# fx-erick/uncertainty-vit

Hardware: AMD Instinct MI355X
Metric: pretrain images/sec (ViT-B/16 224, bs=128/GPU) (higher is better)
Workload: dtype bf16

## Files before the change

include/uvit.h:

```cpp
#ifndef UVIT_H
#define UVIT_H
#include <stddef.h>
#include <stdint.h>

#ifdef __cplusplus
extern "C" {
#endif

#define UVIT_VERSION 100
#define UVIT_MAX_DEPTH 64

typedef struct uvit_engine uvit_engine;
typedef void* uvit_stream;

typedef struct uvit_config {
    int32_t img_size, patch_size, in_chans, embed_dim, depth, num_heads, mlp_hidden;
    int32_t use_shared_rel_pos_bias;
    int32_t use_abs_pos_emb;
    int32_t batch;
    float ln_eps;
    float attn_drop_rate;
    float drop_path_rate;
    int32_t bias_chunk;
    int32_t two_stream;
// ... 91 lines not shown

typedef struct uvit_gemm_epilogue {
    void* out; void* out2; const float* bias; const float* bias2; const float* gamma; const float* resid;
    const float* rowscale; const void* aux; const int64_t* mask; const float* mask_token;
    int32_t ldo, tokens, patches;
    int32_t row0;
} uvit_gemm_epilogue;
enum { UVIT_EPI_BF16 = 0, UVIT_EPI_QKV = 1, UVIT_EPI_GELU = 2, UVIT_EPI_RESID = 3, UVIT_EPI_F32 = 4,
       UVIT_EPI_PATCH = 5, UVIT_EPI_DGELU = 6, UVIT_EPI_QKV_ELU = 7,
       UVIT_EPI_GELU_DG = 8,
       UVIT_EPI_MULAUX = 9 };

int uvit_op_gemm_nt(int mode, const void* A_bf16, const void* W_bf16, int M, int N, int K, int lda, int ldw,
                    const uvit_gemm_epilogue* epi, uvit_stream stream);
int uvit_op_gemm_nt_tuned(int mode, const void* A_bf16, const void* W_bf16, int M, int N, int K, int lda, int ldw,
                          const uvit_gemm_epilogue* epi, const uvit_tuning* tune, int* tail_rows, uvit_stream stream);
typedef struct uvit_gemm_nt_plan_info { int32_t kernel, rows, grid, tail_rows; } uvit_gemm_nt_plan_info;
int uvit_op_gemm_nt_plan(int mode, int M, int N, int K, int lda, int ldw, int ldo, int row_list,
                         const uvit_tuning* tuning, int num_cu, uvit_gemm_nt_plan_info* out);
int uvit_op_gemm_nt_sched(int mode, const void* A_bf16, const void* W_bf16, int M, int N, int K, int lda, int ldw,
                          const uvit_gemm_epilogue* epi, const uvit_tuning* tune, uint32_t* tile_counters, uvit_stream stream);
int uvit_op_gemm_tn(const void* Y_bf16, const void* X_bf16, int M, int N, int K, int ldy, int ldx, float* C, int ldc,
                    const uvit_tuning* tune, uvit_stream stream);
typedef struct uvit_wgrad_problem {
    const void* Y_bf16; const void* X_bf16; float* C; float* bias; float* bias2;
    int32_t bias_end, bias2_begin, M, N, K, ldy, ldx, ldc;
} uvit_wgrad_problem;
int uvit_op_wgrad_group(const uvit_wgrad_problem* problems, int count, const uvit_tuning* tune, uvit_stream stream);
int uvit_op_attn_fwd(const void* qkv, const float* biasP, void* out, float* lse, int B, int H, int N, int NP,
                     float scale, float p_drop, uint32_t seed, uint32_t layer, uvit_stream stream);
int64_t uvit_op_attn_bwd_ws_bytes(int B, int H, int N);
int uvit_op_attn_bwd(const void* qkv, const void* o_fwd, const void* d_o, const float* biasP, const float* lse,
                           float* delta, void* dqkv, float* dbias_slab, int accumulate_slab, void* ds_workspace, int B, int H,
                           int N, int NP, float scale, float p_drop, uint32_t seed, uint32_t layer, uvit_stream stream);
int uvit_op_attn_fwd_hd(const void* qkv, const float* biasP, void* out, float* lse, int B, int H, int N, int NP, int head_dim,
                        float scale, float p_drop, uint32_t seed, uint32_t layer, uvit_stream stream);
int uvit_op_attn_bwd_hd(const void* qkv, const void* o_fwd, const void* d_o, const float* biasP, const float* lse,
                        float* delta, void* dqkv, float* dbias_slab, int accumulate_slab, void* ds_workspace, int B, int H,
                        int N, int NP, int head_dim, float scale, float p_drop, uint32_t seed, uint32_t layer, uvit_stream stream);
int uvit_op_attn2_fwd(const void* qkv_m, const void* qkv_c, const float* biasP, void* out_m, void* out_c, float* lse, int B, int H,
                      int N, int NP, float scale, float p_drop, uint32_t seed, uint32_t layer, uvit_stream stream);
int64_t uvit_op_attn2_bwd_ws_bytes(int B, int H, int N);
int uvit_op_attn2_bwd(const void* qkv_m, const void* qkv_c, const void* o_m, const void* o_c, const void* d_m, const void* d_c,
                      const float* biasP, const float* lse, float* delta, void* dqkv_m, void* dqkv_c, float* dbias_slab,
                      int accumulate_slab, void* ds_workspace, int B, int H, int N, int NP, float scale, float p_drop, uint32_t seed,
                      uint32_t layer, uvit_stream stream);
int uvit_op_relpos_gather(const float* table, const int32_t* index, float* biasP, int H, int N, int NP, uvit_stream stream);
int uvit_op_relpos_scatter(const float* slab, int nslab, const int32_t* index, float* dtable, int H, int N, int NP,
                           uvit_stream stream);
int uvit_op_ln_fwd(const float* x, const float* w, const float* b, void* y_bf16, float* mean, float* rstd, int M, int C,
                   float eps, uvit_stream stream);
int uvit_op_ln_bwd(const void* dy_bf16, const float* x, const float* mean, const float* rstd, const float* w,
                   const float* dres, float* dx, float* dw, float* db, int M, int C, uvit_stream stream);
int uvit_op_ema(float* ema, const float* params, void* ema_bf16, int64_t n, float decay, uvit_stream stream);
int uvit_op_sumsq(const float* g, int64_t n, double* out, uvit_stream stream);
int uvit_op_adamw(float* p, const float* g, float* m, float* v, void* p_bf16, int64_t n, int64_t n_decay, float lr,
                  float wd, float b1, float b2, float eps, int step, const double* sumsq, float max_norm,
                  float grad_scale, float* gnorm_out, uvit_stream stream);
int uvit_op_smooth_l1(const float* out, const float* target, const int32_t* count_dev, float beta, int l2,
                      float loss_scale, float* loss, void* dout_bf16, int Mmax, int C, uvit_stream stream);
int uvit_op_wasserstein_loss(const float* out_m, const float* out_c, const float* tgt_m, const float* tgt_c,
                             const int32_t* count_dev, float lam, float loss_scale, float* scratch, float* loss,
                             void* dout_m_bf16, void* dout_c_bf16, int Mmax, int C, uvit_stream stream);
int uvit_op_target_accum(const float* x, const int32_t* rowidx, const int32_t* count, float* acc, int first, int Mmax,
                         int C, float eps, uvit_stream stream);
int uvit_op_variance_loss(const float* out, const int32_t* count_dev, float w, float margin, float loss_scale, float* scratch,
                          float* loss, float* std_loss0_out, void* dout_bf16, int Mmax, int C, uvit_stream stream);
int uvit_op_target_finalize(float* acc, const int32_t* count, int n_layers, int post_ln, int Mmax, int C, float eps,
                            uvit_stream stream);
int uvit_op_mask_compact(const int64_t* mask, int32_t* rowidx, int32_t* count, int B, int P, uvit_stream stream);
int uvit_op_synth_batch(float* images, int64_t* mask, int B, int chans, int img_size, int patches, int n_mask, uint32_t seed,
                        uint32_t it, uvit_stream stream);
int uvit_op_im2col(const float* img, void* cols_bf16, int B, int Cin, int img_size, int patch, uvit_stream stream);
int uvit_op_droppath(float* scales, const float* rates_dev, int depth, int B, uint32_t seed, uint32_t step,
                     uvit_stream stream);
int uvit_op_cast_bf16(const float* src, void* dst_bf16, int64_t n, uvit_stream stream);

#define UVIT_AUG_LANCZOS 1
#define UVIT_AUG_BILINEAR 2
#define UVIT_AUG_BICUBIC 3
#define UVIT_AUG_HAMMING 5
#define UVIT_AUG_BRIGHTNESS 0
#define UVIT_AUG_CONTRAST 1
#define UVIT_AUG_SATURATION 2
typedef struct uvit_augment_desc {
    int64_t offset;
    int32_t h, w;
    int32_t flip;
    int32_t crop_x, crop_y, crop_w, crop_h;
    int32_t resize_w, resize_h;
    int32_t win_x, win_y;
    int32_t filter;
    int32_t n_jitter;
    int32_t jitter_op[3];
    float jitter_factor[3];
    int32_t reserved;
} uvit_augment_desc;
int64_t uvit_op_augment_ws_bytes(const uvit_augment_desc* desc, int B, int S);
int uvit_op_augment_batch(const uint8_t* pixels, int64_t pixel_bytes, const uvit_augment_desc* desc, int B, int S, const float* mean,
                          const float* std, float* out, void* workspace, int64_t ws_bytes, uvit_stream stream);

int64_t uvit_op_probe_pool_ws_bytes(int B, int N, int C);
int uvit_op_probe_pool_norm(const float* x, float* feat, float* scratch, int B, int N, int C, float eps, uvit_stream stream);
int uvit_op_probe_logits(const float* feat, const float* W, const float* bias, float* logits, int B, int K, int C, uvit_stream stream);
int uvit_op_probe_ce(const float* logits, const int64_t* labels, float smoothing, float* dlogits, float* row_loss, float* loss_out,
                     int32_t* top1_top5, int B, int K, uvit_stream stream);
// ... 15 lines not shown
```

uncertainty-vit_amd/csrc/engine.hip:

```cpp
#include <hip/hip_runtime.h>
#include <math.h>
#include <stdio.h>
#include <stdlib.h>
#include <string.h>

#include <string>
#include <vector>

#include "../../include/uvit.h"
#include "common.h"
#include "uvit_internal.h"

#define CHECK(x) do { int _rc = (x); if (_rc) return _rc; } while (0)
#define NREP 32
#define RP(off) (e->grep + ((off) - e->lo.n_decay))
#define HIPCHECK(x) do { if ((x) != hipSuccess) return UVIT_ERR_LAUNCH; } while (0)
#define GEMM_NT(...) uvit_gemm_nt_launch(__VA_ARGS__, &e->tune)
#define GEMM_TN(...) uvit_gemm_tn_launch(__VA_ARGS__, &e->tune)
#define GEMM_TN_GROUP(...) uvit_gemm_tn_group_launch(__VA_ARGS__, &e->tune)

struct LayerOff { size_t n1w, n1b, qkvw, qb[2], vb[2], projw[2], projb[2], g1, n2w, n2b, fc1w, fc1b, fc2w, fc2b, g2, cqkvw; };
struct Layout {
    size_t cls[2], mask_tok[2], pew[2], peb[2], relt, normw, normb, lmw[2], lmb[2], pos;
    LayerOff L[UVIT_MAX_DEPTH];
    size_t n_total, n_decay, n_live;
    std::vector<uvit_layout_entry> entries;
};

static size_t align64(size_t x) { return (x + 63) & ~(size_t)63; }

static int cfg_ok(const uvit_config* c) {
    if (!c) return UVIT_ERR_ARG;
    if (c->depth < 1 || c->depth > UVIT_MAX_DEPTH || c->num_heads < 1) return UVIT_ERR_SHAPE;
    if (c->embed_dim != c->num_heads * 64 && (c->two_stream || c->embed_dim != c->num_heads * 80)) return UVIT_ERR_SHAPE;
    if (c->embed_dim % 64 || c->mlp_hidden % 64 || c->patch_size % 8 || c->img_size % c->patch_size) return UVIT_ERR_SHAPE;
    if ((c->in_chans * c->patch_size * c->patch_size) % 64) return UVIT_ERR_SHAPE;
    const int g = c->img_size / c->patch_size;
    if (g * g + 1 > 208 || c->batch < 1) return UVIT_ERR_SHAPE;
    if (c->use_abs_pos_emb && c->two_stream) return UVIT_ERR_SHAPE;
    return UVIT_OK;
}

static void build_layout(const uvit_config* c, Layout& lo) {
    const int64_t C = c->embed_dim, Hd = c->mlp_hidden, g = c->img_size / c->patch_size;
    size_t off = 0;
    auto add = [&](const std::string& name, std::vector<int64_t> shape, int decay) -> size_t {
        uvit_layout_entry e;
        memset(&e, 0, sizeof(e));
        snprintf(e.name, sizeof(e.name), "%s", name.c_str());
        e.offset = (int64_t)off; e.ndim = (int)shape.size(); e.decay = decay; e.numel = 1;
        for (size_t i = 0; i < shape.size(); ++i) { e.shape[i] = shape[i]; e.numel *= shape[i]; }
        lo.entries.push_back(e);
        const size_t at = off;
        off = align64(off + (size_t)e.numel);
        return at;
    };
    auto blk = [](int i, const char* s) { return "blocks." + std::to_string(i) + "." + s; };
    const bool two = c->two_stream != 0;
    lo.mask_tok[0] = add("mask_token", {1, 1, C}, 1);
    if (two) lo.mask_tok[1] = add("cov_mask_token", {1, 1, C}, 1);
    if (two) lo.cls[1] = add("cov_cls_token", {1, 1, C}, 1);
    if (c->use_shared_rel_pos_bias) lo.relt = add("rel_pos_bias.relative_position_bias_table", {(2 * g - 1) * (2 * g - 1) + 3, c->num_heads}, 1);
    else lo.relt = (size_t)-1;
    lo.pew[0] = add("patch_embed.proj.weight", {C, c->in_chans, c->patch_size, c->patch_size}, 1);
// ... 1050 lines not shown
    return UVIT_OK;
}
extern "C" int uvit_op_attn_fwd_hd(const void* qkv, const float* biasP, void* out, float* lse, int B, int H, int N, int NP, int head_dim,
                                   float scale, float p_drop, uint32_t seed, uint32_t layer, uvit_stream st) {
    if (!qkv || !out || !lse) return UVIT_ERR_ARG;
    if (head_dim != 64 && head_dim != 80) return UVIT_ERR_SHAPE;
    return uvit_attn_fwd_launch(qkv, biasP, out, lse, B, H, N, NP, scale, p_drop, seed, layer, S(st), nullptr, head_dim);
}
extern "C" int uvit_op_attn_bwd_hd(const void* qkv, const void* o_fwd, const void* d_o, const float* biasP, const float* lse,
                                   float* delta, void* dqkv, float* slab, int acc, void* ds_ws, int B, int H, int N, int NP, int head_dim,
                                   float scale, float p_drop, uint32_t seed, uint32_t layer, uvit_stream st) {
    if (!qkv || !o_fwd || !d_o || !lse || !delta || !dqkv || (slab && !ds_ws)) return UVIT_ERR_ARG;
    if (head_dim != 64 && head_dim != 80) return UVIT_ERR_SHAPE;
    CHECK(uvit_attn_bwd_fused_launch(qkv, o_fwd, d_o, biasP, lse, delta, dqkv, ds_ws, slab != nullptr, B, H, N, NP, scale, p_drop, seed, layer,
                                     S(st), nullptr, head_dim));
    if (slab) CHECK(uvit_attn_dbias_reduce_launch(ds_ws, slab, acc, B, H, N, NP, S(st)));
    return UVIT_OK;
}
extern "C" int uvit_op_attn2_fwd(const void* qkv_m, const void* qkv_c, const float* biasP, void* out_m, void* out_c, float* lse, int B,
                                 int H, int N, int NP, float scale, float p_drop, uint32_t seed, uint32_t layer, uvit_stream st) {
    if (!qkv_m || !qkv_c || !out_m || !out_c || !lse) return UVIT_ERR_ARG;
    return uvit_attn2_fwd_launch(qkv_m, qkv_c, biasP, out_m, out_c, lse, B, H, N, NP, scale, p_drop, seed, layer, S(st));
}
extern "C" int64_t uvit_op_attn2_bwd_ws_bytes(int B, int H, int N) {
    if (B <= 0 || H <= 0 || N <= 0) return UVIT_ERR_SHAPE;
    return (int64_t)uvit_attn2_bwd_ws_bytes(B, H, N);
}
extern "C" int uvit_op_attn2_bwd(const void* qkv_m, const void* qkv_c, const void* o_m, const void* o_c, const void* d_m, const void* d_c,
                                 const float* biasP, const float* lse, float* delta, void* dqkv_m, void* dqkv_c, float* slab, int acc,
                                 void* ds_ws, int B, int H, int N, int NP, float scale, float p_drop, uint32_t seed, uint32_t layer,
                                 uvit_stream st) {
    if (!qkv_m || !qkv_c || !o_m || !o_c || !d_m || !d_c || !lse || !delta || !dqkv_m || !dqkv_c || (slab && !ds_ws)) return UVIT_ERR_ARG;
    CHECK(uvit_attn2_bwd_launch(qkv_m, qkv_c, o_m, o_c, d_m, d_c, biasP, lse, delta, dqkv_m, dqkv_c, ds_ws, slab != nullptr, B, H, N, NP,
                                scale, p_drop, seed, layer, S(st)));
    if (slab) CHECK(uvit_attn2_dbias_reduce_launch(ds_ws, slab, acc, B, H, N, NP, S(st)));
    return UVIT_OK;
}
extern "C" int uvit_op_relpos_gather(const float* t, const int32_t* idx, float* biasP, int H, int N, int NP, uvit_stream st) {
    return uvit_relpos_gather_launch(t, idx, biasP, H, N, NP, S(st));
}
extern "C" int uvit_op_relpos_scatter(const float* slab, int nslab, const int32_t* idx, float* dt, int H, int N, int NP, uvit_stream st) {
    return uvit_relpos_scatter_launch(slab, nslab, idx, dt, H, N, NP, S(st));
}
extern "C" int uvit_op_ln_fwd(const float* x, const float* w, const float* b, void* y, float* mean, float* rstd, int M, int C,
                              float eps, uvit_stream st) {
    LnFwd p; p.x = x; p.w = w; p.b = b; p.y = (bf16*)y; p.mean = mean; p.rstd = rstd; p.M = M; p.C = C; p.eps = eps;
    return uvit_ln_fwd_launch(p, S(st));
}
extern "C" int uvit_op_ln_bwd(const void* dy, const float* x, const float* mean, const float* rstd, const float* w,
                              const float* dres, float* dx, float* dw, float* db, int M, int C, uvit_stream st) {
    LnBwd p; p.dy = (const bf16*)dy; p.x = x; p.mean = mean; p.rstd = rstd; p.w = w; p.dres = dres; p.dx = dx; p.dw = dw; p.db = db; p.M = M; p.C = C;
    return uvit_ln_bwd_launch(p, S(st));
}
extern "C" int uvit_op_ema(float* ema, const float* p, void* eb, int64_t n, float d, uvit_stream st) {
    return uvit_ema_launch(ema, p, eb, (size_t)n, d, S(st));
}
extern "C" int uvit_op_sumsq(const float* g, int64_t n, double* out, uvit_stream st) { return uvit_sumsq_launch(g, (size_t)n, out, S(st)); }
extern "C" int uvit_op_adamw(float* p, const float* g, float* m, float* v, void* pb, int64_t n, int64_t nd, float lr, float wd,
                             float b1, float b2, float eps, int step, const double* sumsq, float max_norm, float gs,
                             float* gn, uvit_stream st) {
    return uvit_adamw_launch(p, g, m, v, pb, (size_t)n, (size_t)nd, lr, wd, b1, b2, eps, step, sumsq, max_norm, gs, gn, S(st));
}
extern "C" int uvit_op_smooth_l1(const float* out, const float* target, const int32_t* count, float beta, int l2, float ls,
                                 float* loss, void* dout, int Mmax, int C, uvit_stream st) {
    return uvit_smooth_l1_launch(out, target, count, beta, l2, ls, loss, dout, Mmax, C, S(st));
}
extern "C" int uvit_op_wasserstein_loss(const float* om, const float* oc, const float* tm, const float* tc, const int32_t* count, float lam,
                                        float ls, float* scratch, float* loss, void* dm, void* dc, int Mmax, int C, uvit_stream st) {
    if (!om || !oc || !tm || !tc || !count || !scratch || !loss || !dm || !dc || Mmax < 1 || C < 1) return UVIT_ERR_ARG;
    return uvit_wasserstein_loss_launch(om, oc, tm, tc, count, lam, ls, scratch, loss, dm, dc, Mmax, C, S(st));
}
extern "C" int uvit_op_variance_loss(const float* out, const int32_t* count, float w, float margin, float ls, float* scratch, float* loss,
                                     float* std_out, void* dout, int Mmax, int C, uvit_stream st) {
    if (!out || !count || !scratch || !loss || !dout) return UVIT_ERR_ARG;
    return uvit_variance_loss_launch(out, count, w, margin, ls, scratch, loss, std_out, dout, Mmax, C, S(st));
}
extern "C" int uvit_op_target_accum(const float* x, const int32_t* rowidx, const int32_t* count, float* acc, int first, int Mmax,
                                    int C, float eps, uvit_stream st) {
    return uvit_target_accum_launch(x, rowidx, count, acc, first, Mmax, C, eps, S(st));
}
extern "C" int uvit_op_target_finalize(float* acc, const int32_t* count, int nl, int post_ln, int Mmax, int C, float eps, uvit_stream st) {
    return uvit_target_finalize_launch(acc, count, nl, post_ln, Mmax, C, eps, S(st));
}
extern "C" int uvit_op_mask_compact(const int64_t* mask, int32_t* rowidx, int32_t* count, int B, int P, uvit_stream st) {
    return uvit_mask_compact_launch(mask, rowidx, count, B, P, S(st));
}
extern "C" int uvit_op_synth_batch(float* images, int64_t* mask, int B, int chans, int img_size, int patches, int n_mask, uint32_t seed,
                                   uint32_t it, uvit_stream st) {
    if (!images && !mask) return UVIT_ERR_ARG;
    return uvit_synth_batch_launch(images, mask, B, chans, img_size, patches, n_mask, seed, it, S(st));
}
extern "C" int uvit_op_im2col(const float* img, void* cols, int B, int Cin, int S_, int p, uvit_stream st) {
    return uvit_im2col_launch(img, cols, B, Cin, S_, p, S(st));
}
extern "C" int uvit_op_droppath(float* sc, const float* rates, int depth, int B, uint32_t seed, uint32_t step, uvit_stream st) {
    return uvit_droppath_launch(sc, rates, depth, 2, B, seed, step, S(st));
}
extern "C" int uvit_op_cast_bf16(const float* src, void* dst, int64_t n, uvit_stream st) { return uvit_cast_bf16_launch(src, dst, (size_t)n, S(st)); }
```

uncertainty-vit_amd/csrc/norm.hip:

```cpp
#include "common.h"
#include "uvit_internal.h"
#include "rowwise.h"

#define LN_WAVES 4

enum LnWalk { WALK_ROWS, WALK_SAMPLES };

template <int NV, LnWalk WALK>
__global__ __launch_bounds__(LN_WAVES * 64)
void ln_fwd_kernel(const float* __restrict__ x, const int* __restrict__ rowidx, const int* __restrict__ count,
                   const int* __restrict__ pos, const float* __restrict__ w, const float* __restrict__ b, bf16* __restrict__ y,
                   float* __restrict__ mean_o, float* __restrict__ rstd_o, float* __restrict__ xcopy, int M, int C, float eps, int tokens) {
    const int lane = threadIdx.x & 63;
    const int row = blockIdx.x * LN_WAVES + (threadIdx.x >> 6);
    if (row >= M) return;
    const int nv = C >> 2;
    int src = row;
    size_t dst = row;
    if constexpr (WALK == WALK_ROWS) {
        if (row >= (count ? *count : M)) { store_zero_row<NV>(y + (size_t)row * C, nv, lane); return; }
        if (rowidx) src = rowidx[row];
    }
    RowVec<NV> r;
    load_row(r, x + (size_t)src * C, C, lane);
    if constexpr (WALK == WALK_SAMPLES) {
        const int smp = row / tokens, slot = pos[smp];
        if (slot < 0) {
#pragma unroll
            for (int k = 0; k < NV; ++k) if (lane + 64 * k < nv) ((float4*)(xcopy + (size_t)row * C))[lane + 64 * k] = r.v[k];
            return;
        }
        dst = (size_t)slot * tokens + (row - smp * tokens);
    }
    float mean, rstd;
    row_stats(r, C, lane, eps, mean, rstd);
    if (lane == 0 && (WALK == WALK_SAMPLES || mean_o)) { mean_o[dst] = mean; rstd_o[dst] = rstd; }
    normalize_store(r, mean, rstd, w, b, y + dst * C, nv, lane);
}

#define LNB_WAVES 8

template <int NV, bool LS>
struct LnbRow {
    float4 x[NV], dres[NV];
    bf16x4 dy[NV], y[LS ? NV : 1];
    float mean, rstd, dp;
    int xr;
    int ar;
    int yr;
};

template <int NV, LnWalk WALK, bool LS>
__device__ __forceinline__ void lnb_load(LnbRow<NV, LS>& r, int row, const bf16* dy, const float* x, const int* map,
                                         const float* mean_i, const float* rstd_i, const float* dres, const LsNext& ls,
                                         int C, int nv, int lane) {
    const int tokens = ls.tokens;
    r.dp = 1.0f;
    if constexpr (WALK == WALK_ROWS) {
        const int xr = map ? map[row] : row;
        r.xr = xr; r.ar = row; r.yr = xr;
        r.mean = mean_i[row]; r.rstd = rstd_i[row];
        if constexpr (LS) {
            if (ls.rowscale) r.dp = ls.rowscale[xr / tokens];
            if (ls.pos) { const int smp = xr / tokens, sl = ls.pos[smp]; r.yr = sl < 0 ? -1 : sl * tokens + (xr - smp * tokens); }
        }
    } else {
        const int smp = row / tokens, t = row - smp * tokens;
        const int sa = map ? map[smp] : smp, sb = LS ? (ls.pos ? ls.pos[smp] : smp) : -1;
        r.xr = row;
        r.ar = sa < 0 ? -1 : sa * tokens + t;
        r.yr = sb < 0 ? -1 : sb * tokens + t;
        r.mean = 0.f; r.rstd = 0.f;
        if (r.ar >= 0) { r.mean = mean_i[r.ar]; r.rstd = rstd_i[r.ar]; }
        if (r.yr >= 0 && ls.rowscale) r.dp = ls.rowscale[smp];
    }
#pragma unroll
    for (int k = 0; k < NV; ++k) {
        const int i = lane + 64 * k;
        if (i < nv) {
            if (WALK == WALK_ROWS || r.ar >= 0) {
                r.x[k] = ((const float4*)(x + (size_t)r.xr * C))[i];
                r.dy[k] = ((const bf16x4*)(dy + (size_t)r.ar * C))[i];
            }
            r.dres[k] = WALK == WALK_SAMPLES || dres ? ((const float4*)(dres + (size_t)r.xr * C))[i] : make_float4(0.f, 0.f, 0.f, 0.f);
            if constexpr (LS) if (WALK == WALK_ROWS || r.yr >= 0) r.y[k] = ((const bf16x4*)(ls.y + (size_t)r.xr * C))[i];
        }
    }
}

template <int NV>
__device__ __forceinline__ void lnb_pad_fill(const LsNext& ls, int C, int nv, int lane, int wave) {
    const int n = *ls.cnt, npad = ((ls.pad_base + n + 63) & ~63) - ls.pad_base;
    for (int r = n + wave; r < npad; r += LNB_WAVES) {
        store_zero_row<NV>(ls.dy + (size_t)r * C, nv, lane);
        if (ls.pad2) for (int c = lane * 4; c < ls.pad2_cols; c += 256) *(bf16x4*)(ls.pad2 + (size_t)r * ls.pad2_cols + c) = bf16x4_zero();
    }
}

template <int NV, LnWalk WALK, bool LS>
__global__ __launch_bounds__(LNB_WAVES * 64)
void ln_bwd_kernel(const bf16* __restrict__ dy, const float* __restrict__ x, const int* __restrict__ map ,
                   const int* __restrict__ count, const float* __restrict__ mean_i, const float* __restrict__ rstd_i,
                   const float* __restrict__ w, const float* __restrict__ dres, float* __restrict__ dx,
                   float* __restrict__ dw, float* __restrict__ db, int M, int C, int nrep, size_t rep_stride, LsNext ls,
                   int rows_per_block) {
    __shared__ float red[LNB_WAVES][64 * 4];
    const int lane = threadIdx.x & 63, wave = threadIdx.x >> 6;
    const int nv = C >> 2;
    int n_valid = M;
    if constexpr (WALK == WALK_ROWS) { if (count) n_valid = min(*count, M); }
    if constexpr (WALK == WALK_SAMPLES && LS) { if (ls.cnt && blockIdx.x == gridDim.x - 1) lnb_pad_fill<NV>(ls, C, nv, lane, wave); }
    float4 ww[NV], gm[LS ? NV : 1];
    RowVec<NV> aw, ab;
    RowVec<LS ? NV : 1> ag, ay;
#pragma unroll
    for (int k = 0; k < NV; ++k) {
        aw.v[k] = make_float4(0.f, 0.f, 0.f, 0.f); ab.v[k] = aw.v[k];
        ww[k] = lane + 64 * k < nv ? ((const float4*)w)[lane + 64 * k] : aw.v[k];
    }
#pragma unroll
    for (int k = 0; k < (LS ? NV : 1); ++k) {
        ag.v[k] = make_float4(0.f, 0.f, 0.f, 0.f); ay.v[k] = ag.v[k]; gm[k] = ag.v[k];
        if constexpr (LS) { if (lane + 64 * k < nv) gm[k] = ((const float4*)ls.gamma)[lane + 64 * k]; }
    }
    const int row_end = min((int)(blockIdx.x + 1) * rows_per_block, n_valid);
    int row = blockIdx.x * rows_per_block + wave;
    LnbRow<NV, LS> cur, nxt;
    if (row < row_end) lnb_load<NV, WALK, LS>(cur, row, dy, x, map, mean_i, rstd_i, dres, ls, C, nv, lane);
    for (; row < row_end; row += LNB_WAVES) {
        const bool more = row + LNB_WAVES < row_end;
        if (more) lnb_load<NV, WALK, LS>(nxt, row + LNB_WAVES, dy, x, map, mean_i, rstd_i, dres, ls, C, nv, lane);
        const bool own = WALK == WALK_ROWS || cur.ar >= 0;
        const float mean = cur.mean, rstd = cur.rstd;
        float4 g[NV], h[NV];
        float s1 = 0.f, s2 = 0.f;
        if (own) {
#pragma unroll
            for (int k = 0; k < NV; ++k) {
                if (lane + 64 * k < nv) {
                    const float d0 = bf2f(cur.dy[k][0]), d1 = bf2f(cur.dy[k][1]), d2 = bf2f(cur.dy[k][2]), d3 = bf2f(cur.dy[k][3]);
                    h[k] = normalize4(cur.x[k], mean, rstd);
                    aw.v[k].x += d0 * h[k].x; aw.v[k].y += d1 * h[k].y; aw.v[k].z += d2 * h[k].z; aw.v[k].w += d3 * h[k].w;
                    ab.v[k].x += d0; ab.v[k].y += d1; ab.v[k].z += d2; ab.v[k].w += d3;
                    g[k] = make_float4(d0 * ww[k].x, d1 * ww[k].y, d2 * ww[k].z, d3 * ww[k].w);
                    s1 += g[k].x + g[k].y + g[k].z + g[k].w;
                    s2 += g[k].x * h[k].x + g[k].y * h[k].y + g[k].z * h[k].z + g[k].w * h[k].w;
                } else {
                    g[k] = make_float4(0.f, 0.f, 0.f, 0.f); h[k] = g[k];
                }
            }
            s1 = wave_sum(s1) / C;
            s2 = wave_sum(s2) / C;
        }
#pragma unroll
        for (int k = 0; k < NV; ++k) {
            const int i = lane + 64 * k;
            if (i < nv) {
                float4 o = cur.dres[k];
                if (own) o = make_float4(o.x + rstd * (g[k].x - s1 - h[k].x * s2), o.y + rstd * (g[k].y - s1 - h[k].y * s2),
                                         o.z + rstd * (g[k].z - s1 - h[k].z * s2), o.w + rstd * (g[k].w - s1 - h[k].w * s2));
                ((float4*)(dx + (size_t)cur.xr * C))[i] = o;
                if constexpr (LS) if (cur.yr >= 0)
                    ls_apply(o, cur.dp, cur.y[k], gm[k], (bf16x4*)(ls.dy + (size_t)cur.yr * C) + i, ag.v[k], ay.v[k]);
            }
        }
        if (more) cur = nxt;
    }
    const size_t rep = (size_t)(blockIdx.x % nrep) * rep_stride;
    auto fold = [&](const float4& part, float* dst, int k) {
        __syncthreads();
        ((float4*)red[wave])[lane] = part;
        __syncthreads();
        if (lane < 32) {
            const int col = wave * 32 + lane;
            float sum = 0.f;
#pragma unroll
            for (int q = 0; q < LNB_WAVES; ++q) sum += red[q][col];
            const int c = 256 * k + col;
            if (c < C) atomicAdd(dst + rep + c, sum);
        }
    };
#pragma unroll
    for (int k = 0; k < NV; ++k) {
        if (64 * k < nv) {
            fold(aw.v[k], dw, k);
            fold(ab.v[k], db, k);
            if constexpr (LS) { fold(ag.v[k], ls.dgamma, k); fold(ay.v[k], ls.dbias, k); }
        }
    }
}

template <int NV>
__global__ __launch_bounds__(LN_WAVES * 64)
void target_accum_kernel(const float* __restrict__ x, const float* __restrict__ sub, const int* __restrict__ rowidx,
                         const int* __restrict__ count, float* __restrict__ acc, int first, int Mmax, int C, float eps, int ln) {
    const int lane = threadIdx.x & 63;
    const int row = blockIdx.x * LN_WAVES + (threadIdx.x >> 6);
    if (row >= Mmax) return;
    const int nv = C >> 2;
    float4* dst = (float4*)(acc + (size_t)row * C);
    if (row >= *count) {
        if (first)
#pragma unroll
            for (int k = 0; k < NV; ++k) if (lane + 64 * k < nv) dst[lane + 64 * k] = make_float4(0.f, 0.f, 0.f, 0.f);
        return;
    }
    RowVec<NV> r;
    load_row(r, x + (size_t)rowidx[row] * C, C, lane);
    if (sub) {
        RowVec<NV> q;
        load_row(q, sub + (size_t)rowidx[row] * C, C, lane);
#pragma unroll
        for (int k = 0; k < NV; ++k) { r.v[k].x -= q.v[k].x; r.v[k].y -= q.v[k].y; r.v[k].z -= q.v[k].z; r.v[k].w -= q.v[k].w; }
    }
    float mean = 0.f, rstd = 1.f;
    if (ln) row_stats(r, C, lane, eps, mean, rstd);
    normalize_store(r, mean, rstd, (float*)dst, !first, nv, lane);
}

template <int NV>
__global__ __launch_bounds__(LN_WAVES * 64)
void target_finalize_kernel(float* __restrict__ acc, const int* __restrict__ count, float inv_layers, int post_ln,
                            int Mmax, int C, float eps) {
    const int lane = threadIdx.x & 63;
    const int row = blockIdx.x * LN_WAVES + (threadIdx.x >> 6);
    if (row >= Mmax || row >= *count) return;
    const int nv = C >> 2;
    RowVec<NV> r;
    load_row(r, acc + (size_t)row * C, C, lane);
#pragma unroll
    for (int k = 0; k < NV; ++k) { r.v[k].x *= inv_layers; r.v[k].y *= inv_layers; r.v[k].z *= inv_layers; r.v[k].w *= inv_layers; }
    float mean = 0.f, rstd = 1.f;
    if (post_ln) row_stats(r, C, lane, eps, mean, rstd);
    normalize_store(r, mean, rstd, acc + (size_t)row * C, false, nv, lane);
}

#define LNB_BLOCKS_PER_CU 1
static int lnb_rows(int M, int resident_blocks_per_cu) {
    static int ncu = 0;
    if (!ncu) {
        int dev = 0; hipDeviceProp_t prop;
        ncu = (hipGetDevice(&dev) == hipSuccess && hipGetDeviceProperties(&prop, dev) == hipSuccess && prop.multiProcessorCount > 0)
                  ? prop.multiProcessorCount : 256;
    }
    const int target = ncu * resident_blocks_per_cu;
    int rows = (M + target - 1) / target;
    rows = ((rows + LNB_WAVES - 1) / LNB_WAVES) * LNB_WAVES;
    return rows < LNB_WAVES ? LNB_WAVES : rows;
}

static int ln_shape_ok(int M, int C) { return (M > 0 && C > 0 && (C % 4) == 0 && C <= ROW_MAXV * 256) ? UVIT_OK : UVIT_ERR_SHAPE; }
static dim3 ln_grid(int M) { return dim3((M + LN_WAVES - 1) / LN_WAVES); }

int uvit_ln_fwd_launch(const LnFwd& p, hipStream_t s) {
    const bool samples = p.pos || p.xcopy;
    if (ln_shape_ok(p.M, p.C) || (samples && (p.rowidx || p.count))) return UVIT_ERR_SHAPE;
    if (samples && (p.tokens <= 0 || (p.M % p.tokens) || !p.pos || !p.xcopy || !p.mean || !p.rstd)) return UVIT_ERR_SHAPE;
    dispatch_nv(p.C, [&](auto nv) {
        constexpr int NV = decltype(nv)::value;
        hipLaunchKernelGGL((samples ? ln_fwd_kernel<NV, WALK_SAMPLES> : ln_fwd_kernel<NV, WALK_ROWS>), ln_grid(p.M), dim3(LN_WAVES * 64), 0, s,
                           p.x, p.rowidx, p.count, p.pos, p.w, p.b, p.y, p.mean, p.rstd, p.xcopy, p.M, p.C, p.eps, p.tokens);
    });
    return uvit_check_launch();
}
int uvit_ln_bwd_launch(const LnBwd& p, hipStream_t s) {
    const LsNext& n = p.next;
    const bool ls = n.dy != nullptr, samples = p.pos || n.cnt || (n.pos && !p.rowidx);
    if (ln_shape_ok(p.M, p.C) || (p.rowidx && !p.count) || (samples && (p.rowidx || p.count))) return UVIT_ERR_SHAPE;
    if ((ls || samples) && n.tokens <= 0) return UVIT_ERR_SHAPE;
    if (samples && ((p.M % n.tokens) || !p.dres)) return UVIT_ERR_SHAPE;
    if (((n.pos || n.cnt) && !ls) || n.pad_base < 0 || (n.pad2 && (!n.cnt || n.pad2_cols <= 0 || (n.pad2_cols % 4)))) return UVIT_ERR_SHAPE;
    const int rpb = lnb_rows(p.M, LNB_BLOCKS_PER_CU);
    dispatch_nv(p.C, [&](auto nv) {
        constexpr int NV = decltype(nv)::value;
        auto kernel = samples ? (ls ? ln_bwd_kernel<NV, WALK_SAMPLES, true> : ln_bwd_kernel<NV, WALK_SAMPLES, false>)
                              : (ls ? ln_bwd_kernel<NV, WALK_ROWS, true> : ln_bwd_kernel<NV, WALK_ROWS, false>);
        hipLaunchKernelGGL(kernel, dim3((p.M + rpb - 1) / rpb), dim3(LNB_WAVES * 64), 0, s, p.dy, p.x, samples ? p.pos : p.rowidx, p.count,
                           p.mean, p.rstd, p.w, p.dres, p.dx, p.dw, p.db, p.M, p.C, p.nrep > 0 ? p.nrep : 1, p.rep_stride, n, rpb);
    });
    return uvit_check_launch();
}
int uvit_target_accum_launch(const float* x, const int* rowidx, const int* count, float* acc, int first, int Mmax,
                             int C, float eps, hipStream_t s, const float* sub, int ln) {
    if (ln_shape_ok(Mmax, C)) return UVIT_ERR_SHAPE;
    dispatch_nv(C, [&](auto nv) {
        hipLaunchKernelGGL(target_accum_kernel<decltype(nv)::value>, ln_grid(Mmax), dim3(LN_WAVES * 64), 0, s, x, sub, rowidx, count, acc, first,
                           Mmax, C, eps, ln);
    });
    return uvit_check_launch();
}
int uvit_target_finalize_launch(float* acc, const int* count, int n_layers, int post_ln, int Mmax, int C, float eps,
                                hipStream_t s) {
    if (ln_shape_ok(Mmax, C) || n_layers <= 0) return UVIT_ERR_SHAPE;
    dispatch_nv(C, [&](auto nv) {
        hipLaunchKernelGGL(target_finalize_kernel<decltype(nv)::value>, ln_grid(Mmax), dim3(LN_WAVES * 64), 0, s, acc, count, 1.0f / n_layers,
                           post_ln, Mmax, C, eps);
    });
    return uvit_check_launch();
}

__global__ __launch_bounds__(256)
void reduce_replicas_kernel(const float* __restrict__ rep, float* __restrict__ out, size_t n4, int nrep, size_t stride4) {
    for (size_t i = blockIdx.x * (size_t)blockDim.x + threadIdx.x; i < n4; i += (size_t)gridDim.x * blockDim.x) {
        float4 a = ((const float4*)out)[i];
        for (int r = 0; r < nrep; ++r) {
            const float4 b = ((const float4*)rep)[(size_t)r * stride4 + i];
            a.x += b.x; a.y += b.y; a.z += b.z; a.w += b.w;
        }
        ((float4*)out)[i] = a;
    }
}
int uvit_reduce_replicas_launch(const float* rep, float* out, size_t n, int nrep, size_t stride, hipStream_t s) {
    if (n % 4 || stride % 4) return UVIT_ERR_SHAPE;
    size_t g = (n / 4 + 255) / 256;
    hipLaunchKernelGGL(reduce_replicas_kernel, dim3((unsigned)(g > 1024 ? 1024 : g)), dim3(256), 0, s, rep, out, n / 4, nrep, stride / 4);
    return uvit_check_launch();
}

__global__ __launch_bounds__(256)
void gather_patch_rows_kernel(const float* __restrict__ x, const float* __restrict__ sub, float* __restrict__ v, int B, int P, int C4) {
    const size_t total = (size_t)B * P * C4;
    for (size_t i = blockIdx.x * (size_t)blockDim.x + threadIdx.x; i < total; i += (size_t)gridDim.x * blockDim.x) {
        const size_t row = i / C4; const int c = (int)(i - row * C4);
        const int b = (int)(row / P), p_ = (int)(row - (size_t)b * P);
        const size_t src = ((size_t)b * (P + 1) + 1 + p_) * C4 + c;
        float4 a = ((const float4*)x)[src];
        if (sub) { const float4 q = ((const float4*)sub)[src]; a.x -= q.x; a.y -= q.y; a.z -= q.z; a.w -= q.w; }
        ((float4*)v)[i] = a;
    }
}

// ... 71 lines not shown
```

uncertainty-vit_amd/native.py:

```python
import ctypes as C
import os
import subprocess

import torch

_HERE = os.path.dirname(os.path.abspath(__file__))
LIB_PATH = os.path.join(_HERE, "libuvit.so")
MAX_DEPTH = 64


class UvitError(RuntimeError):
    pass


_ERR = {-1: "bad argument", -2: "unsupported shape", -3: "HIP launch/runtime error", -4: "workspace too small"}


def check(rc, what=""):
    if rc != 0:
        raise UvitError(f"libuvit: {what} failed: {_ERR.get(rc, rc)} ({rc})")


class Config(C.Structure):
    _fields_ = [(n, C.c_int32) for n in ("img_size", "patch_size", "in_chans", "embed_dim", "depth", "num_heads",
# ... 62 lines not shown
               [("jitter_op", C.c_int32 * 3), ("jitter_factor", C.c_float * 3), ("reserved", C.c_int32)]


_vp, _i, _i64, _f, _u32 = C.c_void_p, C.c_int, C.c_int64, C.c_float, C.c_uint32
_PROTOTYPES = {
    "uvit_version": (_i, []),
    "uvit_source_hash": (C.c_char_p, []),
    "uvit_layout_count": (_i, [_vp]),
    "uvit_layout_get": (_i, [_vp, _i, _vp]),
    "uvit_arena_numel": (_i64, [_vp, _vp]),
    "uvit_workspace_bytes": (_i64, [_vp]),
    "uvit_engine_create": (_vp, [_vp, _vp, _vp, _vp]),
    "uvit_engine_destroy": (None, [_vp]),
    "uvit_engine_sync_shadows": (_i, [_vp, _i, _vp]),
    "uvit_engine_forward_features": (_i, [_vp, _i, _vp, _vp, _i, _i, _u32, _u32, _vp]),
    "uvit_engine_head": (_i, [_vp, _i, _i, _vp, _vp, _vp]),
    "uvit_engine_ws_ptr": (_vp, [_vp, C.c_char_p, _i]),
    "uvit_engine_compact_rows": (_i, [_vp]),
    "uvit_step_begin": (_i, [_vp, _vp, _vp, _vp, _vp]),
    "uvit_step_backward_layer": (_i, [_vp, _i, _vp, _vp]),
    "uvit_step_backward_embed": (_i, [_vp, _vp]),
    "uvit_step_wait_layer_grads": (_i, [_vp, _i, _vp]),
    "uvit_step_update": (_i, [_vp, _vp, _vp]),
    "uvit_train_step": (_i, [_vp, _vp, _vp, _vp, _vp]),
    "uvit_engine_read_stats": (_i, [_vp, _vp, _vp]),
    "uvit_engine_read_stats_async": (_i, [_vp, _vp, _vp]),
    "uvit_tuning_default": (None, [_vp]),
    "uvit_engine_set_tuning": (_i, [_vp, _vp]),
    "uvit_op_wgrad_group": (_i, [_vp, _i, _vp, _vp]),
    "uvit_engine_set_streams": (_i, [_vp, _i]),
    "uvit_engine_set_drop_path_rows": (_i, [_vp, _i]),
    "uvit_drop_path_kept_counts": (_i, [_i, _f, _i, _i, _u32, _u32, _vp]),
    "uvit_engine_profile": (_i, [_vp, _i, _i]),
    "uvit_engine_profile_read": (_i, [_vp, _vp, _vp, _vp]),
    "uvit_engine_profile_read_kind": (_i, [_vp, _i, _vp, _vp, _vp, _vp]),
    "uvit_op_gemm_nt": (_i, [_i, _vp, _vp, _i, _i, _i, _i, _i, _vp, _vp]),
    "uvit_op_gemm_nt_tuned": (_i, [_i, _vp, _vp, _i, _i, _i, _i, _i, _vp, _vp, _vp, _vp]),
    "uvit_op_gemm_nt_plan": (_i, [_i, _i, _i, _i, _i, _i, _i, _i, _vp, _i, _vp]),
    "uvit_op_gemm_nt_sched": (_i, [_i, _vp, _vp, _i, _i, _i, _i, _i, _vp, _vp, _vp, _vp]),
    "uvit_op_gemm_tn": (_i, [_vp, _vp, _i, _i, _i, _i, _i, _vp, _i, _vp, _vp]),
    "uvit_op_wasserstein_loss": (_i, [_vp, _vp, _vp, _vp, _vp, _f, _f, _vp, _vp, _vp, _vp, _i, _i, _vp]),
    "uvit_op_attn_fwd": (_i, [_vp, _vp, _vp, _vp, _i, _i, _i, _i, _f, _f, _u32, _u32, _vp]),
    "uvit_op_attn_bwd_ws_bytes": (_i64, [_i, _i, _i]),
    "uvit_op_attn_bwd": (_i, [_vp, _vp, _vp, _vp, _vp, _vp, _vp, _vp, _i, _vp, _i, _i, _i, _i, _f, _f, _u32, _u32, _vp]),
    "uvit_op_attn_fwd_hd": (_i, [_vp, _vp, _vp, _vp, _i, _i, _i, _i, _i, _f, _f, _u32, _u32, _vp]),
    "uvit_op_attn_bwd_hd": (_i, [_vp, _vp, _vp, _vp, _vp, _vp, _vp, _vp, _i, _vp, _i, _i, _i, _i, _i, _f, _f, _u32, _u32, _vp]),
    "uvit_op_attn2_fwd": (_i, [_vp, _vp, _vp, _vp, _vp, _vp, _i, _i, _i, _i, _f, _f, _u32, _u32, _vp]),
    "uvit_op_attn2_bwd_ws_bytes": (_i64, [_i, _i, _i]),
    "uvit_op_attn2_bwd": (_i, [_vp] * 12 + [_i, _vp, _i, _i, _i, _i, _f, _f, _u32, _u32, _vp]),
    "uvit_op_relpos_gather": (_i, [_vp, _vp, _vp, _i, _i, _i, _vp]),
    "uvit_op_relpos_scatter": (_i, [_vp, _i, _vp, _vp, _i, _i, _i, _vp]),
    "uvit_op_ln_fwd": (_i, [_vp, _vp, _vp, _vp, _vp, _vp, _i, _i, _f, _vp]),
    "uvit_op_ln_bwd": (_i, [_vp, _vp, _vp, _vp, _vp, _vp, _vp, _vp, _vp, _i, _i, _vp]),
    "uvit_op_ema": (_i, [_vp, _vp, _vp, _i64, _f, _vp]),
    "uvit_op_sumsq": (_i, [_vp, _i64, _vp, _vp]),
    "uvit_op_adamw": (_i, [_vp, _vp, _vp, _vp, _vp, _i64, _i64, _f, _f, _f, _f, _f, _i, _vp, _f, _f, _vp, _vp]),
    "uvit_op_smooth_l1": (_i, [_vp, _vp, _vp, _f, _i, _f, _vp, _vp, _i, _i, _vp]),
    "uvit_op_target_accum": (_i, [_vp, _vp, _vp, _vp, _i, _i, _i, _f, _vp]),
    "uvit_op_variance_loss": (_i, [_vp, _vp, _f, _f, _f, _vp, _vp, _vp, _vp, _i, _i, _vp]),
    "uvit_op_target_finalize": (_i, [_vp, _vp, _i, _i, _i, _i, _f, _vp]),
    "uvit_op_mask_compact": (_i, [_vp, _vp, _vp, _i, _i, _vp]),
    "uvit_op_im2col": (_i, [_vp, _vp, _i, _i, _i, _i, _vp]),
    "uvit_op_synth_batch": (_i, [_vp, _vp, _i, _i, _i, _i, _i, _u32, _u32, _vp]),
    "uvit_op_droppath": (_i, [_vp, _vp, _i, _i, _u32, _u32, _vp]),
    "uvit_op_cast_bf16": (_i, [_vp, _vp, _i64, _vp]),
    "uvit_op_augment_ws_bytes": (_i64, [_vp, _i, _i]),
    "uvit_op_augment_batch": (_i, [_vp, _i64, _vp, _i, _i, _vp, _vp, _vp, _vp, _i64, _vp]),
    "uvit_op_probe_pool_ws_bytes": (_i64, [_i, _i, _i]),
    "uvit_op_probe_pool_norm": (_i, [_vp, _vp, _vp, _i, _i, _i, _f, _vp]),
    "uvit_op_probe_logits": (_i, [_vp, _vp, _vp, _vp, _i, _i, _i, _vp]),
    "uvit_op_probe_ce": (_i, [_vp, _vp, _f, _vp, _vp, _vp, _vp, _i, _i, _vp]),
    "uvit_op_probe_head_grad": (_i, [_vp, _vp, _vp, _vp, _i, _i, _i, _vp]),
    "uvit_op_calib_softmax": (_i, [_vp, _vp, _i, _i, _vp]),
    "uvit_op_calib_confidence": (_i, [_vp, _vp, _vp, _i, _i, _vp, _vp, _vp, _vp, _vp, _i, _i, _vp]),
    "uvit_op_calib_tace": (_i, [_vp, _vp, C.c_double, _i, _i, _vp, _vp, _i, _i, _vp]),
    "uvit_op_calib_auroc": (_i, [_vp, _vp, _vp, _vp, _i, _i, _vp]),
}
SYMBOLS = list(_PROTOTYPES)

_lib = None


def source_hash():
    import hashlib
    src = os.path.join(_HERE, "csrc")
    h = hashlib.sha256()
    for f in sorted(n for n in os.listdir(src) if n.endswith((".hip", ".h"))):
        with open(os.path.join(src, f), "rb") as fh:
            h.update(fh.read())
    with open(os.path.join(_HERE, "..", "include", "uvit.h"), "rb") as fh:
        h.update(fh.read())
    return h.hexdigest()[:16]


def build(force=False):
    if os.path.exists(LIB_PATH) and not force:
        try:
            with open(LIB_PATH + ".hash") as fh:
                if fh.read().strip() == source_hash():
                    return LIB_PATH
        except OSError:
            pass
    subprocess.run(["bash", os.path.join(_HERE, "csrc", "build.sh"), LIB_PATH], check=True)
    return LIB_PATH


# ... 49 lines not shown
```

Baseline: 5417.

## Balance LayerNorm backward row partition and batch the weight-grad reduction

The LN backward kernel now splits rows across blocks with a proportional slab partition (one block per CU when rows are plentiful), replacing the fixed rows-per-block rounding that could leave blocks unevenly loaded. The final dw/db (and layer-scale) reduction now stages several accumulator vectors in LDS at once and reduces them with all waves, rather than doing one sync-heavy fold per vector. It also adds walk-variant C entry points, a partition query, and optional timestamp instrumentation compiled only under LN_STAMP. The trade-offs are a larger LDS footprint per block and possibly more atomic traffic per block.

Result: no change. 5474, median of 6 (+1.0%).

```diff
diff --git a/include/uvit.h b/include/uvit.h
--- a/include/uvit.h
+++ b/include/uvit.h
@@ -167,6 +167,16 @@
                    float eps, uvit_stream stream);
 int uvit_op_ln_bwd(const void* dy_bf16, const float* x, const float* mean, const float* rstd, const float* w,
                    const float* dres, float* dx, float* dw, float* db, int M, int C, uvit_stream stream);
+int uvit_op_ln_fwd_walk(const float* x, const float* w, const float* b, void* y_bf16, float* mean, float* rstd, int M, int C,
+                        float eps, const int32_t* rowidx, const int32_t* count, const int32_t* pos, float* xcopy, int tokens,
+                        uvit_stream stream);
+int uvit_op_ln_bwd_walk(const void* dy_bf16, const float* x, const float* mean, const float* rstd, const float* w,
+                        const float* dres, float* dx, float* dw, float* db, int M, int C, int nrep, int64_t rep_stride,
+                        const int32_t* rowidx, const int32_t* count, const int32_t* pos, const void* ls_y_bf16,
+                        const float* ls_gamma, const float* ls_rowscale, void* ls_dy_bf16, float* ls_dgamma, float* ls_dbias,
+                        int tokens, const int32_t* ls_pos, const int32_t* ls_cnt, int pad_base, void* pad2_bf16, int pad2_cols,
+                        uvit_stream stream);
+int uvit_op_ln_partition(int n, int ncu, int32_t* bounds, int cap);
 int uvit_op_ema(float* ema, const float* params, void* ema_bf16, int64_t n, float decay, uvit_stream stream);
 int uvit_op_sumsq(const float* g, int64_t n, double* out, uvit_stream stream);
 int uvit_op_adamw(float* p, const float* g, float* m, float* v, void* p_bf16, int64_t n, int64_t n_decay, float lr,
diff --git a/uncertainty-vit_amd/csrc/engine.hip b/uncertainty-vit_amd/csrc/engine.hip
--- a/uncertainty-vit_amd/csrc/engine.hip
+++ b/uncertainty-vit_amd/csrc/engine.hip
@@ -10,6 +10,7 @@
 #include "../../include/uvit.h"
 #include "common.h"
 #include "uvit_internal.h"
+#include "ln_partition.h"
 
 #define CHECK(x) do { int _rc = (x); if (_rc) return _rc; } while (0)
 #define NREP 32
@@ -1166,6 +1167,34 @@
     LnBwd p; p.dy = (const bf16*)dy; p.x = x; p.mean = mean; p.rstd = rstd; p.w = w; p.dres = dres; p.dx = dx; p.dw = dw; p.db = db; p.M = M; p.C = C;
     return uvit_ln_bwd_launch(p, S(st));
 }
+extern "C" int uvit_op_ln_fwd_walk(const float* x, const float* w, const float* b, void* y, float* mean, float* rstd, int M, int C,
+                                   float eps, const int32_t* rowidx, const int32_t* count, const int32_t* pos, float* xcopy, int tokens,
+                                   uvit_stream st) {
+    if (!x || !w || !b || !y) return UVIT_ERR_ARG;
+    LnFwd p; p.x = x; p.w = w; p.b = b; p.y = (bf16*)y; p.mean = mean; p.rstd = rstd; p.M = M; p.C = C; p.eps = eps;
+    p.rowidx = rowidx; p.count = count; p.pos = pos; p.xcopy = xcopy; p.tokens = tokens;
+    return uvit_ln_fwd_launch(p, S(st));
+}
+extern "C" int uvit_op_ln_bwd_walk(const void* dy, const float* x, const float* mean, const float* rstd, const float* w,
+                                   const float* dres, float* dx, float* dw, float* db, int M, int C, int nrep, int64_t rep_stride,
+                                   const int32_t* rowidx, const int32_t* count, const int32_t* pos, const void* ls_y,
+                                   const float* ls_gamma, const float* ls_rowscale, void* ls_dy, float* ls_dgamma, float* ls_dbias,
+                                   int tokens, const int32_t* ls_pos, const int32_t* ls_cnt, int pad_base, void* pad2, int pad2_cols,
+                                   uvit_stream st) {
+    if (!dy || !x || !mean || !rstd || !w || !dx || !dw || !db || rep_stride < 0) return UVIT_ERR_ARG;
+    if (ls_dy && (!ls_y || !ls_gamma || !ls_dgamma || !ls_dbias)) return UVIT_ERR_ARG;
+    LnBwd p; p.dy = (const bf16*)dy; p.x = x; p.mean = mean; p.rstd = rstd; p.w = w; p.dres = dres; p.dx = dx; p.dw = dw; p.db = db; p.M = M; p.C = C;
+    p.nrep = nrep; p.rep_stride = (size_t)rep_stride; p.rowidx = rowidx; p.count = count; p.pos = pos;
+    LsNext& n = p.next;
+    n.y = (const bf16*)ls_y; n.gamma = ls_gamma; n.rowscale = ls_rowscale; n.dy = (bf16*)ls_dy; n.dgamma = ls_dgamma; n.dbias = ls_dbias;
+    n.tokens = tokens; n.pos = ls_pos; n.cnt = ls_cnt; n.pad_base = pad_base; n.pad2 = (bf16*)pad2; n.pad2_cols = pad2_cols;
+    return uvit_ln_bwd_launch(p, S(st));
+}
+extern "C" int uvit_op_ln_partition(int n, int ncu, int32_t* bounds, int cap) {
+    const int G = ln_slab_grid(n, ncu);
+    if (bounds && cap > G) for (int b = 0; b <= G; ++b) bounds[b] = G ? ln_slab_begin(n, G, b) : 0;
+    return G;
+}
 extern "C" int uvit_op_ema(float* ema, const float* p, void* eb, int64_t n, float d, uvit_stream st) {
     return uvit_ema_launch(ema, p, eb, (size_t)n, d, S(st));
 }
diff --git a/uncertainty-vit_amd/csrc/ln_partition.h b/uncertainty-vit_amd/csrc/ln_partition.h
--- /dev/null
+++ b/uncertainty-vit_amd/csrc/ln_partition.h
@@ -0,0 +1,17 @@
+#pragma once
+
+#if defined(__HIPCC__) || defined(__CUDACC__)
+#define LNP_FN __host__ __device__ static inline
+#else
+#define LNP_FN static inline
+#endif
+
+#define LNB_WAVES 8
+
+LNP_FN int ln_slab_grid(int n, int ncu) {
+    if (n < 1 || ncu < 1) return 0;
+    const long long full = (long long)ncu * LNB_WAVES;
+    return n >= full ? ncu : (n + LNB_WAVES - 1) / LNB_WAVES;
+}
+LNP_FN int ln_slab_begin(int n, int G, int b) { return (int)((long long)b * n / G); }
+LNP_FN int ln_slab_wave_rows(int rows, int w) { return rows > w ? (rows - w + LNB_WAVES - 1) / LNB_WAVES : 0; }
diff --git a/uncertainty-vit_amd/csrc/norm.hip b/uncertainty-vit_amd/csrc/norm.hip
--- a/uncertainty-vit_amd/csrc/norm.hip
+++ b/uncertainty-vit_amd/csrc/norm.hip
@@ -1,8 +1,26 @@
 #include "common.h"
 #include "uvit_internal.h"
 #include "rowwise.h"
+#include "ln_partition.h"
 
 #define LN_WAVES 4
+
+#ifdef LN_STAMP
+__device__ unsigned long long g_ln_stamps[1024 * LNB_WAVES * 8];
+#define LN_STAMP_AT(k) do { unsigned long long t_; asm volatile("s_memtime %0\n\ts_waitcnt lgkmcnt(0)" : "=s"(t_) :: "memory"); \
+        if (lane == 0 && blockIdx.x < 1024) g_ln_stamps[(blockIdx.x * LNB_WAVES + wave) * 8 + (k)] = t_; } while (0)
+#define LN_STAMP_DRAIN() asm volatile("s_waitcnt vmcnt(0)" ::: "memory")
+#define LN_STAMP_ID() do { if (lane == 0 && blockIdx.x < 1024) g_ln_stamps[(blockIdx.x * LNB_WAVES + wave) * 8 + 7] = \
+        __builtin_amdgcn_s_getreg(4 | (31 << 11)) | ((unsigned long long)__builtin_amdgcn_s_getreg(20 | (31 << 11)) << 32); } while (0)
+extern "C" int uvit_debug_ln_stamps(unsigned long long* host_out) {
+    return hipMemcpyFromSymbol(host_out, HIP_SYMBOL(g_ln_stamps), sizeof(g_ln_stamps)) == hipSuccess ? 0 : -3;
+}
+#else
+#define LN_STAMP_AT(k)
+#define LN_STAMP_DRAIN()
+#define LN_STAMP_ID()
+#endif
+
 
 enum LnWalk { WALK_ROWS, WALK_SAMPLES };
 
@@ -38,7 +56,7 @@
     normalize_store(r, mean, rstd, w, b, y + dst * C, nv, lane);
 }
 
-#define LNB_WAVES 8
+#define LNB_LDS_VECS 12
 
 template <int NV, bool LS>
 struct LnbRow {
@@ -102,11 +120,14 @@
 void ln_bwd_kernel(const bf16* __restrict__ dy, const float* __restrict__ x, const int* __restrict__ map ,
                    const int* __restrict__ count, const float* __restrict__ mean_i, const float* __restrict__ rstd_i,
                    const float* __restrict__ w, const float* __restrict__ dres, float* __restrict__ dx,
-                   float* __restrict__ dw, float* __restrict__ db, int M, int C, int nrep, size_t rep_stride, LsNext ls,
-                   int rows_per_block) {
-    __shared__ float red[LNB_WAVES][64 * 4];
+                   float* __restrict__ dw, float* __restrict__ db, int M, int C, int nrep, size_t rep_stride, LsNext ls) {
+    constexpr int NACC = LS ? 4 : 2;
+    constexpr int CH = NV * NACC <= LNB_LDS_VECS ? NV : LNB_LDS_VECS / NACC;
+    __shared__ float red[LNB_WAVES][NACC * CH][256];
     const int lane = threadIdx.x & 63, wave = threadIdx.x >> 6;
     const int nv = C >> 2;
+    LN_STAMP_ID();
+    LN_STAMP_AT(0);
     int n_valid = M;
     if constexpr (WALK == WALK_ROWS) { if (count) n_valid = min(*count, M); }
     if constexpr (WALK == WALK_SAMPLES && LS) { if (ls.cnt && blockIdx.x == gridDim.x - 1) lnb_pad_fill<NV>(ls, C, nv, lane, wave); }
@@ -123,8 +144,8 @@
         ag.v[k] = make_float4(0.f, 0.f, 0.f, 0.f); ay.v[k] = ag.v[k]; gm[k] = ag.v[k];
         if constexpr (LS) { if (lane + 64 * k < nv) gm[k] = ((const float4*)ls.gamma)[lane + 64 * k]; }
     }
-    const int row_end = min((int)(blockIdx.x + 1) * rows_per_block, n_valid);
-    int row = blockIdx.x * rows_per_block + wave;
+    const int row_end = ln_slab_begin(n_valid, gridDim.x, blockIdx.x + 1);
+    int row = ln_slab_begin(n_valid, gridDim.x, blockIdx.x) + wave;
     LnbRow<NV, LS> cur, nxt;
     if (row < row_end) lnb_load<NV, WALK, LS>(cur, row, dy, x, map, mean_i, rstd_i, dres, ls, C, nv, lane);
     for (; row < row_end; row += LNB_WAVES) {
@@ -166,28 +187,41 @@
         }
         if (more) cur = nxt;
     }
+    LN_STAMP_AT(1);
+    LN_STAMP_DRAIN();
+    LN_STAMP_AT(2);
     const size_t rep = (size_t)(blockIdx.x % nrep) * rep_stride;
-    auto fold = [&](const float4& part, float* dst, int k) {
+#pragma unroll
+    for (int k0 = 0; k0 < NV; k0 += CH) {
+        if (64 * k0 >= nv) break;
+        if (k0) __syncthreads();
+#pragma unroll
+        for (int kk = 0; kk < CH; ++kk) {
+            const int k = k0 + kk;
+            if (k < NV) {
+                ((float4*)red[wave][0 * CH + kk])[lane] = aw.v[k];
+                ((float4*)red[wave][1 * CH + kk])[lane] = ab.v[k];
+                if constexpr (LS) { ((float4*)red[wave][2 * CH + kk])[lane] = ag.v[k]; ((float4*)red[wave][3 * CH + kk])[lane] = ay.v[k]; }
+            }
+        }
         __syncthreads();
-        ((float4*)red[wave])[lane] = part;
-        __syncthreads();
-        if (lane < 32) {
-            const int col = wave * 32 + lane;
-            float sum = 0.f;
-#pragma unroll
-            for (int q = 0; q < LNB_WAVES; ++q) sum += red[q][col];
+        if (k0 == 0) LN_STAMP_AT(3);
+#pragma unroll
+        for (int v = wave; v < NACC * CH * 4; v += LNB_WAVES) {
+            const int vec = v >> 2, col = (v & 3) * 64 + lane, a = vec / CH, k = k0 + vec % CH;
             const int c = 256 * k + col;
-            if (c < C) atomicAdd(dst + rep + c, sum);
-        }
-    };
-#pragma unroll
-    for (int k = 0; k < NV; ++k) {
-        if (64 * k < nv) {
-            fold(aw.v[k], dw, k);
-            fold(ab.v[k], db, k);
-            if constexpr (LS) { fold(ag.v[k], ls.dgamma, k); fold(ay.v[k], ls.dbias, k); }
-        }
-    }
+            if (k < NV && c < C) {
+                float sum = 0.f;
+#pragma unroll
+                for (int wq = 0; wq < LNB_WAVES; ++wq) sum += red[wq][vec][col];
+                float* dst = a == 0 ? dw : a == 1 ? db : a == 2 ? ls.dgamma : ls.dbias;
+                atomicAdd(dst + rep + c, sum);
+            }
+        }
+    }
+    LN_STAMP_AT(4);
+    LN_STAMP_DRAIN();
+    LN_STAMP_AT(5);
 }
 
 template <int NV>
@@ -235,18 +269,14 @@
     normalize_store(r, mean, rstd, acc + (size_t)row * C, false, nv, lane);
 }
 
-#define LNB_BLOCKS_PER_CU 1
-static int lnb_rows(int M, int resident_blocks_per_cu) {
+static int ln_ncu() {
     static int ncu = 0;
     if (!ncu) {
         int dev = 0; hipDeviceProp_t prop;
         ncu = (hipGetDevice(&dev) == hipSuccess && hipGetDeviceProperties(&prop, dev) == hipSuccess && prop.multiProcessorCount > 0)
                   ? prop.multiProcessorCount : 256;
     }
-    const int target = ncu * resident_blocks_per_cu;
-    int rows = (M + target - 1) / target;
-    rows = ((rows + LNB_WAVES - 1) / LNB_WAVES) * LNB_WAVES;
-    return rows < LNB_WAVES ? LNB_WAVES : rows;
+    return ncu;
 }
 
 static int ln_shape_ok(int M, int C) { return (M > 0 && C > 0 && (C % 4) == 0 && C <= ROW_MAXV * 256) ? UVIT_OK : UVIT_ERR_SHAPE; }
@@ -270,13 +300,12 @@
     if ((ls || samples) && n.tokens <= 0) return UVIT_ERR_SHAPE;
     if (samples && ((p.M % n.tokens) || !p.dres)) return UVIT_ERR_SHAPE;
     if (((n.pos || n.cnt) && !ls) || n.pad_base < 0 || (n.pad2 && (!n.cnt || n.pad2_cols <= 0 || (n.pad2_cols % 4)))) return UVIT_ERR_SHAPE;
-    const int rpb = lnb_rows(p.M, LNB_BLOCKS_PER_CU);
     dispatch_nv(p.C, [&](auto nv) {
         constexpr int NV = decltype(nv)::value;
         auto kernel = samples ? (ls ? ln_bwd_kernel<NV, WALK_SAMPLES, true> : ln_bwd_kernel<NV, WALK_SAMPLES, false>)
                               : (ls ? ln_bwd_kernel<NV, WALK_ROWS, true> : ln_bwd_kernel<NV, WALK_ROWS, false>);
-        hipLaunchKernelGGL(kernel, dim3((p.M + rpb - 1) / rpb), dim3(LNB_WAVES * 64), 0, s, p.dy, p.x, samples ? p.pos : p.rowidx, p.count,
-                           p.mean, p.rstd, p.w, p.dres, p.dx, p.dw, p.db, p.M, p.C, p.nrep > 0 ? p.nrep : 1, p.rep_stride, n, rpb);
+        hipLaunchKernelGGL(kernel, dim3(ln_slab_grid(p.M, ln_ncu())), dim3(LNB_WAVES * 64), 0, s, p.dy, p.x, samples ? p.pos : p.rowidx, p.count,
+                           p.mean, p.rstd, p.w, p.dres, p.dx, p.dw, p.db, p.M, p.C, p.nrep > 0 ? p.nrep : 1, p.rep_stride, n);
     });
     return uvit_check_launch();
 }
diff --git a/uncertainty-vit_amd/native.py b/uncertainty-vit_amd/native.py
--- a/uncertainty-vit_amd/native.py
+++ b/uncertainty-vit_amd/native.py
@@ -138,6 +138,9 @@
     "uvit_op_relpos_scatter": (_i, [_vp, _i, _vp, _vp, _i, _i, _i, _vp]),
     "uvit_op_ln_fwd": (_i, [_vp, _vp, _vp, _vp, _vp, _vp, _i, _i, _f, _vp]),
     "uvit_op_ln_bwd": (_i, [_vp, _vp, _vp, _vp, _vp, _vp, _vp, _vp, _vp, _i, _i, _vp]),
+    "uvit_op_ln_fwd_walk": (_i, [_vp] * 6 + [_i, _i, _f, _vp, _vp, _vp, _vp, _i, _vp]),
+    "uvit_op_ln_bwd_walk": (_i, [_vp] * 9 + [_i, _i, _i, _i64] + [_vp] * 9 + [_i, _vp, _vp, _i, _vp, _i, _vp]),
+    "uvit_op_ln_partition": (_i, [_i, _i, _vp, _i]),
     "uvit_op_ema": (_i, [_vp, _vp, _vp, _i64, _f, _vp]),
     "uvit_op_sumsq": (_i, [_vp, _i64, _vp, _vp]),
     "uvit_op_adamw": (_i, [_vp, _vp, _vp, _vp, _vp, _i64, _i64, _f, _f, _f, _f, _f, _i, _vp, _f, _f, _vp, _vp]),
```
